# nwihardjo/SpaghettiSearch

Hardware: AMD Instinct MI355X
Metric: pagerank_iters_per_sec (higher is better)
Workload: dtype f64

## Files before the change

spaghettisearch_amd/csrc/pagerank.hip:

```cpp
#include "pr_state.hpp"

#include <algorithm>
#include <chrono>
#include <cmath>
#include <memory>

namespace {


template <int GW>
__device__ __forceinline__ double wave_sum_topic(double v) {
#pragma unroll
    for (int off = GW; off < 64; off <<= 1) v += __shfl_xor(v, off, 64);
    return v;
}

__device__ __forceinline__ double zero_row_rank(const PrParams& p, int sweep, double S, double x0) {
    return ((sweep == 0 ? x0 : 0.0) + p.teleport) / S;
}
__device__ __forceinline__ double teleport_of(const PrParams& p, uint32_t lrow, int t) {
    if (!p.memb || !((p.ts_mask >> t) & 1u)) return p.teleport;
    return ((p.memb[lrow] >> t) & 1u) ? p.tin[t] : 0.0;
}
__device__ __forceinline__ double zero_row_rank_ts(const PrParams& p, int sweep, double S, double x0, double tele) {
// ... 1032 lines not shown
            w.beg = in_ptr[w.row] + w.count * SEGW;
            w.end = min(in_ptr[w.row + 1], w.beg + SEGW);
            break;
        case V_QUAD:
        case V_DEG: w.beg = in_ptr[w.row]; w.end = in_ptr[w.row + w.count]; break;
        default: return;
    }
    work[i] = w;
}

__global__ __launch_bounds__(TPB) void k_pr_remap_src(const uint32_t* __restrict__ in_src, uint32_t* __restrict__ out, size_t n_edges, uint32_t pos_nd,
                                                      uint32_t cnt_nd, const uint32_t* __restrict__ outdeg, const uint32_t* __restrict__ sh_deg,
                                                      uint32_t n_shared, uint32_t zrow) {
    for (size_t e = (size_t)blockIdx.x * TPB + threadIdx.x; e < n_edges; e += (size_t)gridDim.x * TPB) {
        uint32_t w = NT_LOAD(&in_src[e]);
        const uint32_t s = w & SRC_MASK;
        if (s >= pos_nd) {
            uint32_t row = zrow;
            if (s < cnt_nd && n_shared) {
                const uint32_t od = outdeg[s];
                uint32_t lo = 0, hi = n_shared;
                while (lo < hi) {
                    const uint32_t mid = (lo + hi) >> 1;
                    if (sh_deg[mid] < od) lo = mid + 1; else hi = mid;
                }
                if (lo < n_shared && sh_deg[lo] == od) row = zrow + 1 + lo;
            }
            w = (w & ~SRC_MASK) | row;
        }
        NT_STORE(w, &out[e]);
    }
}

template <int GW>
__global__ __launch_bounds__(TPB) void k_pr_begin(PrParams p) {
    const int lane = threadIdx.x & 63;
    const int t = lane % GW;
    const double x0 = p.x0[t];
    double* __restrict__ Tw = p.tab_wr[1];
    double csum = 0.0;
    for (uint32_t i = blockIdx.x * TPB + threadIdx.x; i < p.n_shared * (uint32_t)GW; i += gridDim.x * TPB)
        Tw[(size_t)(p.zrow + 1) * GW + i] = p.d * x0 / (double)p.sh_deg[i / GW];
    const size_t n_el = ((size_t)p.sl_nd + p.sl_d) * GW;
    for (size_t i = (size_t)blockIdx.x * TPB + threadIdx.x; i < n_el; i += (size_t)gridDim.x * TPB) {
        const uint32_t lrow = (uint32_t)(i / GW);
        const bool real = lrow < p.sl_nd ? lrow < p.cnt_nd : (lrow - p.sl_nd) < p.cnt_d;
        p.x[i] = real ? x0 : 0.0;
        if (lrow < p.sl_nd) {
            double c = 0.0;
            if (real) c = p.d * x0 / (double)p.outdeg[lrow];
            if ((p.world == 1 || lrow + 2 < p.sl_nd) && lrow < p.tab_rows) Tw[i] = c;
            csum += c;
        }
    }
    block_reduce_and_publish<GW>(p, 0.0, csum, Tw, true);
}

template <int GW>
__global__ void k_pr_finalize(PrParams p, const double* __restrict__ table, int is_begin) {
    if (threadIdx.x != 0 || blockIdx.x != 0) return;
    if (!is_begin && p.ctl->n_active == 0) return;
    double dl[MAXK], cs[MAXK];
    for (int k = 0; k < MAXK; k++) { dl[k] = 0.0; cs[k] = 0.0; }
    for (int r = 0; r < p.world; r++) {
        const size_t base = ((size_t)r * p.sl_nd + (p.sl_nd - 2)) * GW;
        for (int k = 0; k < GW; k++) {
// ... 235 lines not shown
        } else {
            SS_GW_DISPATCH(GW, sweep_occupancy, &per_cu);
        }
        occ_cache[slot] = per_cu < 1 ? 1 : per_cu;
    }
    return occ_cache[slot];
}
int multi_blocks_per_cu(int gw) {
    static std::mutex occ2_mu;
    static int occ_multi[3] = {0, 0, 0};
    std::lock_guard<std::mutex> lk2(occ2_mu);
    int& occ = occ_multi[gw <= 2 ? gw : 0];
    if (!occ) {
        int o = 0;
        if (gw == 1) (void)hipOccupancyMaxActiveBlocksPerMultiprocessor(&o, k_pr_multi_n<1, 1>, TPB, 0);
        else (void)hipOccupancyMaxActiveBlocksPerMultiprocessor(&o, k_pr_multi_n<2, 1>, TPB, 0);
        occ = std::max(o, 1);
    }
    return occ;
}
unsigned grid_for(const ss_ctx* ctx, ss_pr* pr, const PlanOptions& opt, int per_cu, bool vitems, size_t n_items) {
    per_cu = (int)std::max<int64_t>(1, opt.blocks_per_cu == PlanOptions::AUTO ? per_cu : opt.blocks_per_cu);
    const int64_t want = ctx->opt("pr.persistent", 0);
    pr->persist_mode = want == 2 ? 2 : 1;
    pr->persist = pr->nwave && pr->g->world == 1 && !ctx->opt("pr.affine", 0) && want > 0;
    if (pr->persist) {
        const int admit = std::max(1, multi_blocks_per_cu(pr->gw) - 2);
        per_cu = (int)std::max<int64_t>(1, std::min<int64_t>(std::min(admit, std::max(1, per_cu / 2)), ctx->opt("pr.persistent_blocks", 4)));
    }
    return vitems ? (unsigned)std::min<size_t>(std::max<size_t>(1, ss::div_up(n_items, (size_t)WAVES * opt.items_per_wave)), (size_t)ctx->cu_count * per_cu)
                  : (unsigned)std::min<size_t>(n_items, (size_t)ctx->cu_count * 8);
}

void fill_params(ss_pr* pr, const Cut& cut, const PlanOptions& opt, double damping, double eps, int32_t max_iter, int32_t k_topics) {
    const ss_graph* g = pr->g;
    PrParams& p = pr->prm;
    p.in_ptr = g->in_ptr.p;
    p.in_src = g->in_src.p;
    p.outdeg = g->outdeg.p;
    p.x = pr->x.p;
    if (g->world == 1) {
        p.tab_rd[0] = pr->tab0.p; p.tab_wr[0] = pr->tab1.p;
        p.tab_rd[1] = pr->tab1.p; p.tab_wr[1] = pr->tab0.p;
    } else {
        p.tab_rd[0] = p.tab_rd[1] = pr->tab0.p;
        p.tab_wr[0] = p.tab_wr[1] = pr->send.p;
    }
    p.work = pr->work.p;
    p.partials = pr->partials.p;
    p.segpart = pr->segpart.p;
    p.rowticket = pr->rowticket.p;
    p.ctl = pr->ctl.p;
    p.x0 = pr->x0.p;
    p.d = damping;
    p.teleport = 1.0 - damping;
    p.eps = eps;
    p.tele_n = p.teleport * (double)g->n;
    p.max_iter = max_iter;
    p.k_topics = k_topics;
    p.world = g->world;
    p.sl_nd = g->sl_nd;
    p.cnt_nd = g->cnt_nd;
    p.sl_d = g->sl_d;
    p.cnt_d = g->cnt_d;
    p.seg_edges = cut.seg_edges;
    p.n_items = (uint32_t)cut.items.size();
    p.pos_nd = cut.pos_nd;
    p.pos_d = cut.pos_d;
    p.zrow = (uint32_t)g->nd_int;
    p.tab_rows = g->sl_nd;
    p.woff = pr->woff.p;
    p.stagger_div = opt.stagger != 0 ? (uint32_t)std::max(g->ctx->cu_count, 1) : 0u;
    p.stagger_code = opt.stagger >= 10 ? (uint32_t)(opt.stagger - 10) : 0u;
    p.class_order = pack_class_order(opt.class_order);
    p.n_order = pack_n_order(opt.n_class_order);
}

uint64_t fnv1a(const void* q, size_t n, uint64_t h = 0xcbf29ce484222325ull) {
    const unsigned char* b = static_cast<const unsigned char*>(q);
    for (size_t i = 0; i < n; i++) { h ^= b[i]; h *= 0x100000001b3ull; }
    return h;
}
void trace_plan(const ss_pr* pr, const std::vector<WorkItem>& work, const std::vector<uint32_t>& woff) {
    const PrParams& p = pr->prm;
    const double sd[] = {p.d, p.teleport, p.eps, p.tele_n};
    const uint32_t su[] = {(uint32_t)p.max_iter, (uint32_t)p.k_topics, (uint32_t)p.world, p.sl_nd, p.cnt_nd, p.sl_d, p.cnt_d, p.seg_edges, p.n_items,
                           p.pos_nd, p.pos_d, p.ts_mask, p.zrow, p.stagger_div, p.stagger_code, p.class_order, p.n_order};
    fprintf(stderr, "[pr trace] plan: work %016llx (%zu items)  woff %016llx  params %016llx  nblocks %u\n",
            (unsigned long long)fnv1a(work.data(), work.size() * sizeof(WorkItem)), work.size(),
            (unsigned long long)fnv1a(woff.data(), woff.size() * sizeof(uint32_t)),
            (unsigned long long)fnv1a(su, sizeof(su), fnv1a(sd, sizeof(sd))), pr->nblocks);
}

int32_t alloc_tables(ss_pr* pr, hipStream_t st, size_t rows) {
    const ss_graph* g = pr->g;
    ss_ctx* ctx = g->ctx;
    const size_t GW = (size_t)pr->gw;
    SS_HIP(ctx, pr->tab0.alloc(rows * GW));
    SS_HIP(ctx, hipMemsetAsync(pr->tab0.p, 0, std::max<size_t>(pr->tab0.bytes(), 8), st));
    if (g->world == 1) {
        SS_HIP(ctx, pr->tab1.alloc(rows * GW));
        SS_HIP(ctx, hipMemsetAsync(pr->tab1.p, 0, std::max<size_t>(pr->tab1.bytes(), 8), st));
    } else {
        SS_HIP(ctx, pr->send.alloc((size_t)g->sl_nd * GW));
        SS_HIP(ctx, hipMemsetAsync(pr->send.p, 0, std::max<size_t>(pr->send.bytes(), 8), st));
    }
    return SS_OK;
}
int32_t unshare_rows(ss_pr* pr, hipStream_t st) {
    if (!pr->prm.share) return SS_OK;
    const ss_graph* g = pr->g;
    SS_HIP(g->ctx, hipStreamSynchronize(st));
    SS_TRY(alloc_tables(pr, st, (size_t)g->nd_int + 1));
    pr->src_shared.release();
    pr->sh_deg.release();
    PrParams& p = pr->prm;
    p.tab_rd[0] = pr->tab0.p; p.tab_wr[0] = pr->tab1.p;
    p.tab_rd[1] = pr->tab1.p; p.tab_wr[1] = pr->tab0.p;
    p.in_src = g->in_src.p;
    p.sh_deg = nullptr;
    p.n_shared = 0;
    p.share = 0;
    p.zrow = (uint32_t)g->nd_int;
    p.tab_rows = g->sl_nd;
    return SS_OK;
}

#ifdef SS_PR_WAVETIME
FILE* open_dump(const char* name) {
    const char* dir = getenv("SS_PR_WAVETIME_DIR");
    return fopen((std::string(dir && *dir ? dir : ".") + "/" + name).c_str(), "w");
}
void dump_wave_loads(const Cut& cut, const std::vector<double>& cost, const std::vector<uint32_t>& owner, uint32_t nw) {
    FILE* f = open_dump("pr_load.csv");
    if (!f) return;
    std::vector<double> wl(nw, 0.0), wcls((size_t)nw * 6, 0.0);
    for (size_t i = 0; i < cut.items.size(); i++) {
        int kc = 0; while (kc < 5 && i >= cut.vbeg[kc + 1]) kc++;
        wl[owner[i]] += cost[i]; wcls[(size_t)owner[i] * 6 + kc] += cost[i];
    }
    fprintf(f, "wave,load,c0,c1,c2,c3,c4,c5\n");
    for (uint32_t w = 0; w < nw; w++) fprintf(f, "%u,%.2f,%.2f,%.2f,%.2f,%.2f,%.2f,%.2f\n", w, wl[w], wcls[(size_t)w * 6], wcls[(size_t)w * 6 + 1], wcls[(size_t)w * 6 + 2], wcls[(size_t)w * 6 + 3], wcls[(size_t)w * 6 + 4], wcls[(size_t)w * 6 + 5]);
    fclose(f);
}
void dump_wave_times(const ss_pr* pr) {
    if (pr->gw < 8) return;
    (void)hipDeviceSynchronize();
    const uint32_t nwv = std::min<uint32_t>(65536u, pr->nblocks * WAVES);
    std::vector<unsigned long long> h((size_t)nwv * 2);
    if (hipMemcpyFromSymbol(h.data(), HIP_SYMBOL(g_pr_wt), h.size() * sizeof(unsigned long long)) != hipSuccess || !nwv) return;
    unsigned long long t0 = ~0ull;
    for (uint32_t w = 0; w < nwv; w++) t0 = std::min(t0, h[2 * w]);
    std::vector<double> st(nwv), en(nwv);
    for (uint32_t w = 0; w < nwv; w++) { st[w] = (double)(h[2 * w] - t0) / 100.0; en[w] = (double)(h[2 * w + 1] - t0) / 100.0; }
    std::sort(st.begin(), st.end()); std::sort(en.begin(), en.end());
    if (FILE* f = open_dump("pr_wt.csv")) {
        fprintf(f, "wave,start_us,end_us\n");
        for (uint32_t w = 0; w < nwv; w++) fprintf(f, "%u,%.2f,%.2f\n", w, (double)(h[2 * w] - t0) / 100.0, (double)(h[2 * w + 1] - t0) / 100.0);
        fclose(f);
    }
    fprintf(stderr, "[pr wavetime] %u waves: start us median %.1f max %.1f | out of items us min %.1f p10 %.1f median %.1f p90 %.1f p99 %.1f max %.1f\n", nwv,
            st[nwv / 2], st[nwv - 1], en[0], en[nwv / 10], en[nwv / 2], en[nwv * 9 / 10], en[(size_t)nwv * 99 / 100], en[nwv - 1]);
}
#endif

}

extern "C" {

int32_t ss_pr_create(ss_graph* g, double damping, double eps, int32_t max_iter, int32_t k_topics,
                     const int32_t* n_topic, ss_pr** out) {
    if (!g) return SS_ERR_INVALID;
    ss_ctx* ctx = g->ctx;
    std::lock_guard<std::recursive_mutex> lk(ctx->mu);
    if (!out) return ctx->fail(SS_ERR_INVALID, "ss_pr_create: out is NULL");
    *out = nullptr;
    if (k_topics < 1 || !n_topic) return ctx->fail(SS_ERR_INVALID, "ss_pr_create: k_topics < 1 or n_topic NULL");
    if (k_topics > MAXK) return ctx->fail(SS_ERR_UNSUPPORTED, "ss_pr_create: k_topics %d > %d per state (ss_pagerank_run splits larger K)", k_topics, MAXK);
    SS_HIP(ctx, hipSetDevice(ctx->device));
    hipStream_t st = ctx->stream;

    ss_pr* pr = new (std::nothrow) ss_pr();
    if (!pr) return ctx->fail(SS_ERR_OOM, "ss_pr_create: host OOM");
    std::unique_ptr<ss_pr> guard(pr);
    pr->g = g;
    pr->k = k_topics;
    const bool force_narrow = ctx->opt("pr.force_narrow", 0) != 0;
    pr->gw = pick_gw(k_topics, g->nd_int, force_narrow, ctx->opt("pr.narrow_wave", 1) != 0);
    pr->nwave = pr->gw <= 2 && !force_narrow && ctx->opt("pr.narrow_wave", 1) != 0;
    const int GW = pr->gw;
    const bool vitems = GW >= 8 || pr->nwave;
    const int GI = pr->nwave ? 8 : GW;
    const size_t n_local = g->n_local();
    if (((uint64_t)g->nd_int + 1) * GW * 8 >= (1ull << 32))
        return ctx->fail(SS_ERR_UNSUPPORTED, "ss_pr_create: contribution table of %llu rows x %d topics exceeds 4 GiB (shard the graph over more ranks)",
                         (unsigned long long)g->nd_int, GW);

    const bool trace = ctx->opt("pr.trace", 0) != 0;
    auto t_now = [] { return std::chrono::steady_clock::now(); };
    auto t_ms = [](std::chrono::steady_clock::time_point a, std::chrono::steady_clock::time_point b) { return std::chrono::duration<double, std::milli>(b - a).count(); };
    SS_HIP(ctx, pr->x.alloc(n_local * GW));
    bool share = GW >= 8 && g->world == 1 && ctx->opt("pr.affine", 0) == 0 && ctx->opt("pr.share_zero_rows", 1) != 0;
    if (!share) SS_TRY(alloc_tables(pr, st, (size_t)g->nd_int + 1));

    const auto tc0 = t_now();
    const PlanOptions opt = plan_options(ctx, pr, n_local);
    Cut cut = cut_items(g->h_indeg_nd, g->h_indeg_d, g->sl_nd, GI, pr->nwave, opt);
    const uint32_t n_tail = g->cnt_nd - cut.pos_nd;
    struct PinGuard { ss_ctx* c; void* p = nullptr; size_t cap = 0; ~PinGuard() { c->pin_free(p, cap); } } tail_od{ctx};
    if (share && n_tail == 0) {
        share = false;
        SS_TRY(alloc_tables(pr, st, (size_t)g->nd_int + 1));
    }
    if (share) {
        tail_od.p = ctx->pin_alloc((size_t)n_tail * sizeof(uint32_t), &tail_od.cap);
        if (!tail_od.p) return ctx->fail(SS_ERR_OOM, "ss_pr_create: no pinned host memory for %u out-degrees", n_tail);
        SS_HIP(ctx, hipMemcpyAsync(tail_od.p, g->outdeg.p + cut.pos_nd, (size_t)n_tail * sizeof(uint32_t), hipMemcpyDeviceToHost, st));
    }
    const auto tc1 = t_now();
    const int per_cu = sweep_blocks_per_cu(pr);
    const auto tc1a = t_now();
    pr->nblocks = grid_for(ctx, pr, opt, per_cu, vitems, cut.items.size());
    static const std::vector<uint32_t> no_woff;
    const std::vector<uint32_t>* woff = &no_woff;
    if (vitems) {
        const uint32_t nw = pr->nblocks * WAVES;
        const auto td0 = t_now();
        const std::vector<double>& cost = item_costs(cut, g->h_indeg_nd, g->h_indeg_d, g->sl_nd, GI, pr->nwave);
        const auto td0a = t_now();
        std::vector<uint32_t>& owner = deal_items(cut, cost, nw, pr->nwave, opt);
#ifdef SS_PR_WAVETIME
        dump_wave_loads(cut, cost, owner, nw);
#endif
        const auto td1 = t_now();
        if (trace) fprintf(stderr, "[pr trace]   deal: occupancy query %.2f ms, costs %.3f ms, owners %.3f ms\n", t_ms(tc1, tc1a), t_ms(td0, td0a), t_ms(td0a, td1));
        woff = &place_items(cut, owner, nw);
        if (trace) fprintf(stderr, "[pr trace]   deal: placement %.3f ms\n", t_ms(td1, t_now()));
    }
    const std::vector<WorkItem>& items = cut.items;

    g->settle();
    const auto tc2 = t_now();
    SharedRows sh;
    if (share) {
        SS_HIP(ctx, hipStreamSynchronize(st));
        const auto ts0 = t_now();
        sh = plan_shared_rows(static_cast<const uint32_t*>(tail_od.p), n_tail, cut.pos_nd);
        const auto ts1 = t_now();
        SS_TRY(alloc_tables(pr, st, (size_t)sh.table_rows));
        SS_HIP(ctx, pr->sh_deg.alloc(sh.deg.size()));
        SS_HIP(ctx, hipMemcpyAsync(pr->sh_deg.p, sh.deg.data(), sh.deg.size() * sizeof(uint32_t), hipMemcpyHostToDevice, st));
        SS_HIP(ctx, pr->src_shared.alloc(g->e_local));
        if (g->e_local)
            hipLaunchKernelGGL(k_pr_remap_src, dim3((unsigned)std::min<uint64_t>(ss::div_up(g->e_local, TPB), (uint64_t)ctx->cu_count * 16)), dim3(TPB), 0, st,
                               (const uint32_t*)g->in_src.p, pr->src_shared.p, (size_t)g->e_local, cut.pos_nd, g->cnt_nd, (const uint32_t*)g->outdeg.p,
                               (const uint32_t*)pr->sh_deg.p, (uint32_t)sh.deg.size(), sh.zrow);
        if (trace) fprintf(stderr, "[pr trace]   shared rows: %u rows without in-edges -> %zu shared rows (host %.3f ms), table %llu rows\n", n_tail, sh.deg.size(),
                           t_ms(ts0, ts1), (unsigned long long)sh.table_rows);
    }
    SS_HIP(ctx, pr->partials.alloc(((size_t)std::max(pr->nblocks, ss::begin_blocks(pr)) + 8) * 2 * GW));
    SS_HIP(ctx, pr->segpart.alloc((size_t)std::max(cut.nsegs, 1u) * GW));
    SS_HIP(ctx, pr->rowticket.alloc(std::max(cut.nmulti, 1u)));
    SS_HIP(ctx, hipMemsetAsync(pr->rowticket.p, 0, pr->rowticket.bytes(), st));
    SS_HIP(ctx, pr->woff.alloc(std::max<size_t>(woff->size(), 8)));
    if (!woff->empty()) SS_HIP(ctx, hipMemcpyAsync(pr->woff.p, woff->data(), woff->size() * sizeof(uint32_t), hipMemcpyHostToDevice, st));
    SS_HIP(ctx, pr->work.alloc(items.size()));
    SS_HIP(ctx, hipMemcpyAsync(pr->work.p, items.data(), items.size() * sizeof(WorkItem), hipMemcpyHostToDevice, st));
    if (vitems)
        hipLaunchKernelGGL(k_pr_item_ranges, dim3(ss::div_up(items.size(), TPB)), dim3(TPB), 0, st, pr->work.p, (uint32_t)items.size(), (const uint32_t*)g->in_ptr.p);
    SS_HIP(ctx, pr->ctl.alloc(1));
    SS_HIP(ctx, hipMemsetAsync(pr->ctl.p, 0, sizeof(PrCtl), st));
    double h_x0[MAXK];
    for (int k = 0; k < MAXK; k++) h_x0[k] = k < k_topics ? 1.0 / (double)n_topic[k] : 0.0;
    SS_HIP(ctx, pr->x0.alloc(MAXK));
    SS_HIP(ctx, hipMemcpyAsync(pr->x0.p, h_x0, sizeof(h_x0), hipMemcpyHostToDevice, st));
    SS_HIP(ctx, hipStreamSynchronize(st));
    if (trace) fprintf(stderr, "[pr trace] ss_pr_create: build_work %.2f ms (%zu items), edge ranges + deal %.2f ms, alloc + upload %.2f ms\n", t_ms(tc0, tc1), items.size(), t_ms(tc1, tc2), t_ms(tc2, t_now()));
    if (trace) fprintf(stderr, "[pr trace] where the state lives: x %p  tab0 %p  tab1 %p  in_src %p  in_ptr %p  outdeg %p  work %p  woff %p\n", (void*)pr->x.p, (void*)pr->tab0.p,
                       (void*)pr->tab1.p, (void*)g->in_src.p, (void*)g->in_ptr.p, (void*)g->outdeg.p, (void*)pr->work.p, (void*)pr->woff.p);

    fill_params(pr, cut, opt, damping, eps, max_iter, k_topics);
    if (share) {
        PrParams& p = pr->prm;
        p.in_src = pr->src_shared.p;
        p.sh_deg = pr->sh_deg.p;
        p.n_shared = (uint32_t)sh.deg.size();
        p.share = 1;
        p.zrow = sh.zrow;
        p.tab_rows = cut.pos_nd;
    }
    if (trace) trace_plan(pr, items, *woff);
    g->users++;
    *out = guard.release();
    return SS_OK;
}

int32_t ss_pr_set_teleport(ss_pr* pr, const uint64_t* set_ptr, const uint32_t* set_nodes) {
    if (!pr) return SS_ERR_INVALID;
    ss_ctx* ctx = pr->g->ctx;
    std::lock_guard<std::recursive_mutex> lk(ctx->mu);
    SS_HIP(ctx, hipSetDevice(ctx->device));
    if (pr->begun) return ctx->fail(SS_ERR_STATE, "ss_pr_set_teleport: call before ss_pr_begin");
    hipStream_t st = ctx->stream;
    PrParams& p = pr->prm;
    if (!set_ptr) {
        p.memb = nullptr; p.tin = nullptr; p.nz_in = nullptr; p.ts_mask = 0;
        return SS_OK;
    }
    const ss_graph* g = pr->g;
    const int K = pr->k;
    SS_TRY(unshare_rows(pr, st));
    std::vector<uint64_t> h_ptr(K + 1);
    SS_HIP(ctx, ss::copy_in(ctx->stream, h_ptr.data(), set_ptr, (K + 1) * sizeof(uint64_t)));
    if (h_ptr[0] != 0) return ctx->fail(SS_ERR_INVALID, "ss_pr_set_teleport: set_ptr[0] != 0");
    for (int k = 0; k < K; k++)
        if (h_ptr[k + 1] < h_ptr[k]) return ctx->fail(SS_ERR_INVALID, "ss_pr_set_teleport: set_ptr not non-decreasing");
    const uint64_t total = h_ptr[K];
    if (total && !set_nodes) return ctx->fail(SS_ERR_INVALID, "ss_pr_set_teleport: set_nodes is NULL");
    double h_tin[MAXK];
    uint32_t mask = 0;
    for (int k = 0; k < MAXK; k++) {
        h_tin[k] = 0.0;
        if (k < K && h_ptr[k + 1] > h_ptr[k]) {
            mask |= 1u << k;
            h_tin[k] = p.teleport * (double)g->n / (double)(h_ptr[k + 1] - h_ptr[k]);
        }
    }
// ... 35 lines not shown
    SS_HIP(ctx, hipMemcpyAsync(pr->nz_in.p, h_nz, sizeof(h_nz), hipMemcpyHostToDevice, st));
    SS_HIP(ctx, hipStreamSynchronize(st));
    p.memb = pr->memb.p;
    p.tin = pr->tin.p;
    p.nz_in = pr->nz_in.p;
    p.ts_mask = mask;
    return SS_OK;
}

int32_t ss_pr_destroy(ss_pr* pr) {
#ifdef SS_PR_WAVETIME
    if (pr) dump_wave_times(pr);
#endif

    if (!pr) return SS_ERR_INVALID;
    ss_ctx* ctx = pr->g->ctx;
    std::lock_guard<std::recursive_mutex> lk(ctx->mu);
    (void)hipSetDevice(ctx->device);
    if (!ss::device_wedged(ctx->device)) {
        (void)hipStreamSynchronize(ctx->stream);
        (void)hipStreamSynchronize(ctx->comm_stream);
    }
    pr->g->users--;
    delete pr;
    return SS_OK;
}

int32_t ss_pr_begin(ss_pr* pr) {
    if (!pr) return SS_ERR_INVALID;
    ss_ctx* ctx = pr->g->ctx;
    std::lock_guard<std::recursive_mutex> lk(ctx->mu);
    SS_HIP(ctx, hipSetDevice(ctx->device));
    if (pr->need_finalize) return ctx->fail(SS_ERR_STATE, "ss_pr_begin: pending exchange/finalize");
    SS_HIP(ctx, hipMemsetAsync(&pr->ctl.p->ticket, 0, sizeof(uint32_t), ctx->stream));
    ss::pr_launch_begin(pr, ctx->stream, ss::begin_blocks(pr));
    SS_HIP(ctx, hipGetLastError());
    pr->begun = true;
    if (pr->g->world > 1) {
        pr->need_finalize = true;
        pr->finalize_is_begin = true;
    }
    return SS_OK;
}

int32_t ss_pr_step(ss_pr* pr, int32_t n_steps) {
    if (!pr) return SS_ERR_INVALID;
    ss_ctx* ctx = pr->g->ctx;
    std::lock_guard<std::recursive_mutex> lk(ctx->mu);
    SS_HIP(ctx, hipSetDevice(ctx->device));
    if (!pr->begun) return ctx->fail(SS_ERR_STATE, "ss_pr_step: ss_pr_begin not called");
    if (pr->need_finalize) return ctx->fail(SS_ERR_STATE, "ss_pr_step: pending exchange/finalize");
    if (n_steps < 1) return ctx->fail(SS_ERR_INVALID, "ss_pr_step: n_steps < 1");
    if (pr->g->world > 1 && n_steps != 1) return ctx->fail(SS_ERR_INVALID, "ss_pr_step: world>1 needs an exchange after every step");
    SS_HIP(ctx, hipEventRecord(ctx->ev[0][0], ctx->stream));
    if (pr->persist && !pr->prm.memb && !pr->prm.aff) {
        SS_GW_DISPATCH(pr->gw, launch_multi, pr, ctx->stream, (int)n_steps);
    } else {
        for (int i = 0; i < n_steps; i++) ss::pr_launch_step(pr, ctx->stream);
    }
    SS_HIP(ctx, hipEventRecord(ctx->ev[0][1], ctx->stream));
    ctx->ev_valid[0] = true;
    SS_HIP(ctx, hipGetLastError());
    if (pr->g->world > 1) {
        pr->need_finalize = true;
        pr->finalize_is_begin = false;
    }
    return SS_OK;
}

int32_t ss_pr_finalize(ss_pr* pr) {
// ... 156 lines not shown
```

spaghettisearch_amd/csrc/pagerank_run.hip:

```cpp
#include "pr_state.hpp"

#include <algorithm>

namespace {

constexpr int AFF_KC = 16;
__global__ __launch_bounds__(TPB) void k_aff_delta(const double2* __restrict__ xp, const double2* __restrict__ xn, const AffCtl* __restrict__ a,
                                                   uint32_t sl_nd, uint32_t pos_nd, uint32_t pos_d, double* __restrict__ partials) {
    __shared__ double red[WAVES][AFF_KC];
    if (a->n_active == 0) return;
    const int k_real = a->k_real;
    const double r_old = a->r_prev, r_new = a->r_x, s_old = a->s_prev, s_new = a->s_x;
    const uint32_t n_rows = pos_nd + pos_d;
    const int lane = threadIdx.x & 63, wave = threadIdx.x >> 6;
    for (int k0 = 0; k0 < k_real; k0 += AFF_KC) {
        double u[AFF_KC], d_old[AFF_KC], d_new[AFF_KC], acc[AFF_KC];
        bool any = false;
#pragma unroll
        for (int j = 0; j < AFF_KC; j++) {
            const bool on = k0 + j < k_real && a->active[k0 + j] != 0;
            any = any || on;
            u[j] = on ? a->u[k0 + j] : 0.0;
            d_old[j] = on ? r_old * u[j] + s_old : 1.0;
            d_new[j] = on ? r_new * u[j] + s_new : 1.0;
// ... 629 lines not shown
        for (int k = 0; k < k_topics && rc == SS_OK; k++)
            for (size_t i = 0; i < n_rows; i++) rank_out[(size_t)k * n + ids[i]] = part[(size_t)k * n_rows + i];
    }
    for (int s = 0; s < world && rc == SS_OK && !affine; s++) {
        const size_t n_rows = (size_t)shards[s]->cnt_nd + shards[s]->cnt_d;
        std::vector<uint32_t> ids(n_rows);
        for (int b = 0; b < B && rc == SS_OK; b++) {
            const int kb = k0[b + 1] - k0[b];
            std::vector<double> part((size_t)kb * n_rows);
            rc = ss_pr_read_local(sh[s].blk[b], ids.data(), part.data());
            if (rc != SS_OK) break;
            for (int k = 0; k < kb; k++)
                for (size_t i = 0; i < n_rows; i++) rank_out[(size_t)(k0[b] + k) * n + ids[i]] = part[(size_t)k * n_rows + i];
        }
    }
    for (auto& s : sh)
        for (ss_pr* pr : s.blk) ss_pr_destroy(pr);
    return rc;
}

int32_t ss_pagerank_run(ss_graph* g, double damping, double eps, int32_t max_iter, int32_t k_topics,
                        const int32_t* n_topic, double* rank_out, int32_t* iters_out) {
    if (!g) return SS_ERR_INVALID;
    ss_ctx* ctx = g->ctx;
    std::lock_guard<std::recursive_mutex> lk(ctx->mu);
    if (g->world != 1) return ctx->fail(SS_ERR_STATE, "ss_pagerank_run: needs a (rank 0, world 1) graph");
    if (k_topics < 1 || k_topics > SS_MAX_TOPICS || !n_topic || !rank_out)
        return ctx->fail(SS_ERR_INVALID, "ss_pagerank_run: bad k_topics / NULL argument");
    SS_TRY(check_eps(ctx, "ss_pagerank_run", eps, max_iter));
    if (ctx->opt("pr.affine", 0) != 0) return run_affine(g, damping, eps, max_iter, k_topics, n_topic, rank_out, iters_out);
    for (int k0 = 0; k0 < k_topics; k0 += MAXK) {
        const int kk = std::min(MAXK, k_topics - k0);
        ss_pr* pr = nullptr;
        SS_TRY(ss_pr_create(g, damping, eps, max_iter, kk, n_topic + k0, &pr));
        int32_t rc = ss_pr_begin(pr);
        int32_t n_active = kk, sweeps = 0;
        const int BATCH = 8;
        while (rc == SS_OK && n_active > 0) {
            int todo = BATCH;
            if (max_iter > 0) todo = std::min(BATCH, std::max(1, max_iter - sweeps));
            rc = ss_pr_step(pr, todo);
            if (rc == SS_OK) rc = ss_pr_status(pr, iters_out ? iters_out + k0 : nullptr, &n_active, &sweeps, nullptr, nullptr);
        }
        if (rc == SS_OK) rc = ss_pr_read(pr, rank_out + (size_t)k0 * g->n);
        ss_pr_destroy(pr);
        if (rc != SS_OK) return rc;
    }
    return SS_OK;
}

}
```

spaghettisearch_amd/csrc/pr_plan.hpp:

```cpp
#pragma once
#include "sorted_degrees.hpp"

#include <algorithm>
#include <cstdint>
#include <utility>
#include <vector>

namespace {

constexpr int TPB = 256;
constexpr int WAVES = TPB / 64;
constexpr int CH = 16;
constexpr uint32_t SEGW = 2048;

enum : uint32_t { W_SEG = 0, W_WAVE = 1, W_GROUP = 2, W_ZERO = 3,
                  V_SEG = 8,
                  V_ROWW = 9,
                  V_QUAD = 10,
                  V_DEG = 11,
                  V_ZERO = 12 };

struct WorkItem {
    uint32_t kind;
    uint32_t row;
// ... 219 lines not shown
            c0 = c1;
        }
    }
    for (size_t i0 = 0; i0 < n_items; i0 += nw) {
        const size_t n_chunk = std::min<size_t>(nw, n_items - i0);
        if (i0 && snake) {
            std::reverse(by_load.begin(), by_load.end());
        } else if (i0) {
            key.resize(nw);
            for (uint32_t w = 0; w < nw; w++) key[w] = {load[w], w};
            std::sort(key.begin(), key.end());
            for (uint32_t w = 0; w < nw; w++) by_load[w] = key[w].second;
        }
        idx.resize(n_chunk);
        for (size_t j = 0; j < n_chunk; j++) idx[j] = global_order ? order[i0 + j] : (uint32_t)(i0 + j);
        const auto falling = [&](uint32_t a, uint32_t b) { return cost[a] > cost[b]; };
        size_t run_end = 0, n_merge = 0;
        for (size_t j = 1; j <= n_chunk && !global_order; j++) {
            if (j < n_chunk && !(cost[i0 + j] > cost[i0 + j - 1])) continue;
            if (run_end) {
                if (++n_merge > 8) { std::stable_sort(idx.begin(), idx.end(), falling); break; }
                std::inplace_merge(idx.begin(), idx.begin() + (ptrdiff_t)run_end, idx.begin() + (ptrdiff_t)j, falling);
            }
            run_end = j;
        }
        for (size_t j = 0; j < n_chunk; j++) {
            owner[idx[j]] = by_load[j];
            load[by_load[j]] += cost[idx[j]];
        }
    }
    return owner;
}

inline const std::vector<uint32_t>& place_items(Cut& cut, std::vector<uint32_t>& owner, uint32_t nw) {
    PlanScratch& s = plan_scratch();
    auto& items = cut.items;
    auto &woff = s.woff, &cnt = s.cnt;
    woff.assign((size_t)nw * 8, 0);
    cnt.assign((size_t)nw * 8, 0);
    for (int k = 0; k < 6; k++) {
        const size_t i1 = k < 5 ? std::min<size_t>(cut.vbeg[k + 1], items.size()) : items.size();
        for (size_t i = std::min<size_t>(cut.vbeg[k], i1); i < i1; i++) { owner[i] = owner[i] * 8 + (uint32_t)k; cnt[owner[i]]++; }
    }
    uint32_t run_off = 0;
    for (uint32_t w = 0; w < nw; w++) {
        for (int k = 0; k < 8; k++) {
            woff[(size_t)w * 8 + k] = run_off;
            run_off += cnt[(size_t)w * 8 + k];
            cnt[(size_t)w * 8 + k] = woff[(size_t)w * 8 + k];
        }
    }
    s.dealt.resize(items.size());
    for (size_t i = 0; i < items.size(); i++) s.dealt[cnt[owner[i]]++] = items[i];
    s.dealt.push_back({V_ZERO, 0, 0, 0, 0, 0, 0, 0});
    s.dealt.push_back({V_ZERO, 0, 0, 0, 0, 0, 0, 0});
    items.swap(s.dealt);
    return woff;
}

inline uint32_t pack_class_order(int64_t code) {
    uint32_t packed = 0, seen = 0;
    for (int pos = 5; pos >= 0; pos--) {
        const uint32_t c = (uint32_t)(code % 10);
        code /= 10;
        packed |= (c & 7u) << (3 * pos);
        if (c < 6) seen |= 1u << c;
    }
    return seen == 0x3Fu ? packed : (0u | 1u << 3 | 2u << 6 | 3u << 9 | 4u << 12 | 5u << 15);
}
inline uint32_t pack_n_order(int64_t code) {
    uint32_t packed = 0, seen = 0;
    for (int pos = 3; pos >= 0; pos--) {
        const uint32_t c = (uint32_t)(code % 10);
        code /= 10;
        packed |= (c & 3u) << (2 * pos);
        if (c < 4) seen |= 1u << c;
    }
    return seen == 0xFu ? packed : (0u | 1u << 2 | 2u << 4 | 3u << 6);
}

struct SharedRows {
    std::vector<uint32_t> deg;
    uint32_t zrow = 0;
    uint32_t base = 0;
    uint64_t table_rows = 0;
    uint32_t row_of(uint32_t od) const {
        const auto it = std::lower_bound(deg.begin(), deg.end(), od);
        return it != deg.end() && *it == od ? base + (uint32_t)(it - deg.begin()) : zrow;
    }
};
inline SharedRows plan_shared_rows(const uint32_t* od, size_t n, uint32_t pos_nd) {
    SharedRows sh;
    uint32_t hi = 0;
    for (size_t i = 0; i < n; i++) hi = std::max(hi, od[i]);
    if (n && (uint64_t)hi <= 4 * (uint64_t)n + 65536) {
        std::vector<unsigned char> seen((size_t)hi + 1, 0);
        for (size_t i = 0; i < n; i++) seen[od[i]] = 1;
        for (size_t v = 0; v <= hi; v++)
            if (seen[v]) sh.deg.push_back((uint32_t)v);
    } else if (n) {
        sh.deg.assign(od, od + n);
        std::sort(sh.deg.begin(), sh.deg.end());
        sh.deg.erase(std::unique(sh.deg.begin(), sh.deg.end()), sh.deg.end());
    }
    sh.zrow = pos_nd;
    sh.base = pos_nd + 1;
    sh.table_rows = (uint64_t)pos_nd + 1 + sh.deg.size();
    return sh;
}

}
```

spaghettisearch_amd/csrc/pr_state.hpp:

```cpp
#pragma once
#include "graph.hpp"
#include "pr_plan.hpp"

namespace {

constexpr int MAXK = 16;

struct PrCtl {
    double S[MAXK];
    double delta[MAXK];
    double csum[MAXK];
    double xz[MAXK];
    double xz_in[MAXK];
    double tele[MAXK];
    int32_t active[MAXK];
    int32_t iters[MAXK];
    int32_t sweep;
    int32_t n_active;
    uint32_t ticket;
    uint32_t stuck;
    uint32_t gticket[8];
};

constexpr int AFF_MAXK = 256;
// ... 34 lines not shown
    uint32_t stagger_div;
    uint32_t stagger_code;
    uint32_t class_order;
    uint32_t n_order;
    double* x_alt;
    AffCtl* aff;
    const double* tele_col;
    const uint32_t* sh_deg;
    uint32_t n_shared;
    uint32_t share;
    uint32_t tab_rows;
};

}

struct ss_pr {
    ss_graph* g = nullptr;
    int gw = 1;
    ss::DevBuf<float> wire_send, wire_recv;
    bool nwave = false;
    int persist_mode = 1;
    bool persist = false;
    int k = 1;
    PrParams prm{};
    unsigned nblocks = 0;
    ss::DevBuf<double> x, tab0, tab1, send, partials, segpart, x0;
    ss::DevBuf<uint32_t> rowticket;
    ss::DevBuf<uint32_t> memb;
    ss::DevBuf<double> tin, nz_in;
    ss::DevBuf<WorkItem> work;
    ss::DevBuf<uint32_t> woff;
    ss::DevBuf<uint32_t> src_shared;
    ss::DevBuf<uint32_t> sh_deg;
    ss::DevBuf<PrCtl> ctl;
    bool begun = false;
    bool need_finalize = false;
    bool finalize_is_begin = false;
};

#pragma GCC visibility push(hidden)
namespace ss {
unsigned begin_blocks(const ss_pr* pr);
void pr_launch_begin(ss_pr* pr, hipStream_t st, unsigned nb);
void pr_launch_step(ss_pr* pr, hipStream_t st);
void pr_launch_finalize(ss_pr* pr, hipStream_t st, int is_begin);
size_t pr_wire_floats(const ss_pr* pr);
hipError_t pr_wire_alloc(ss_pr* pr);
void pr_wire_pack(ss_pr* pr, hipStream_t st);
void pr_wire_unpack(ss_pr* pr, hipStream_t st);
}
#pragma GCC visibility pop

namespace {
inline int32_t read_ctl(ss_ctx* ctx, const ss_pr* pr, hipStream_t st, const char* what, const PrCtl** out) {
    ctx->pin_used = 0;
    PrCtl* const hp = ctx->pin<PrCtl>();
    if (hipMemcpyAsync(hp, pr->ctl.p, sizeof(PrCtl), hipMemcpyDeviceToHost, st) != hipSuccess) return ctx->fail(SS_ERR_HIP, "%s: status read failed", what);
    SS_TRY(ss::sync_bounded(ctx, st, what));
    *out = hp;
    return SS_OK;
}
}
```

Baseline: 18440.

## Overlap PageRank setup with GPU work and compute tail degrees on device

The create path now builds the set of distinct tail out-degrees with a shared-memory bitmap kernel, so the host reads back a small bitmap instead of every tail out-degree. It falls back to the full copy when a degree is too large for the bitmap. It also enqueues the begin kernel before the host deals work items, writes the plan straight into pinned memory, uploads it asynchronously, and memsets only the unshared part of the rank tables. The goal is to cut host-side setup and synchronisation latency. The cost is more complex lifetime handling for the pinned plan buffer, which the destructor now frees.

New measurement: 18430. Within noise of the previous version (-0.0%).

```diff
diff --git a/spaghettisearch_amd/csrc/pagerank.hip b/spaghettisearch_amd/csrc/pagerank.hip
--- a/spaghettisearch_amd/csrc/pagerank.hip
+++ b/spaghettisearch_amd/csrc/pagerank.hip
@@ -1088,6 +1088,21 @@
     }
 }
 
+constexpr uint32_t SH_SEEN_BITS = 1u << 16, SH_SEEN_WORDS = SH_SEEN_BITS / 32;
+__global__ __launch_bounds__(TPB) void k_pr_tail_degrees(const uint32_t* __restrict__ od, uint32_t n, uint32_t* __restrict__ seen) {
+    __shared__ uint32_t s_seen[SH_SEEN_WORDS + 1];
+    for (uint32_t i = threadIdx.x; i <= SH_SEEN_WORDS; i += TPB) s_seen[i] = 0u;
+    __syncthreads();
+    for (uint32_t i = blockIdx.x * TPB + threadIdx.x; i < n; i += gridDim.x * TPB) {
+        const uint32_t d = od[i];
+        if (d < SH_SEEN_BITS) atomicOr(&s_seen[d >> 5], 1u << (d & 31u));
+        else s_seen[SH_SEEN_WORDS] = 1u;
+    }
+    __syncthreads();
+    for (uint32_t i = threadIdx.x; i <= SH_SEEN_WORDS; i += TPB)
+        if (s_seen[i]) atomicOr(&seen[i], s_seen[i]);
+}
+
 template <int GW>
 __global__ __launch_bounds__(TPB) void k_pr_begin(PrParams p) {
     const int lane = threadIdx.x & 63;
@@ -1389,7 +1404,7 @@
                   : (unsigned)std::min<size_t>(n_items, (size_t)ctx->cu_count * 8);
 }
 
-void fill_params(ss_pr* pr, const Cut& cut, const PlanOptions& opt, double damping, double eps, int32_t max_iter, int32_t k_topics) {
+void fill_params(ss_pr* pr, const Cut& cut, uint32_t n_items, const PlanOptions& opt, double damping, double eps, int32_t max_iter, int32_t k_topics) {
     const ss_graph* g = pr->g;
     PrParams& p = pr->prm;
     p.in_ptr = g->in_ptr.p;
@@ -1421,7 +1436,7 @@
     p.sl_d = g->sl_d;
     p.cnt_d = g->cnt_d;
     p.seg_edges = cut.seg_edges;
-    p.n_items = (uint32_t)cut.items.size();
+    p.n_items = n_items;
     p.pos_nd = cut.pos_nd;
     p.pos_d = cut.pos_d;
     p.zrow = (uint32_t)g->nd_int;
@@ -1438,26 +1453,27 @@
     for (size_t i = 0; i < n; i++) { h ^= b[i]; h *= 0x100000001b3ull; }
     return h;
 }
-void trace_plan(const ss_pr* pr, const std::vector<WorkItem>& work, const std::vector<uint32_t>& woff) {
+void trace_plan(const ss_pr* pr, const WorkItem* work, size_t n_work, const uint32_t* woff, size_t n_woff) {
     const PrParams& p = pr->prm;
     const double sd[] = {p.d, p.teleport, p.eps, p.tele_n};
     const uint32_t su[] = {(uint32_t)p.max_iter, (uint32_t)p.k_topics, (uint32_t)p.world, p.sl_nd, p.cnt_nd, p.sl_d, p.cnt_d, p.seg_edges, p.n_items,
                            p.pos_nd, p.pos_d, p.ts_mask, p.zrow, p.stagger_div, p.stagger_code, p.class_order, p.n_order};
     fprintf(stderr, "[pr trace] plan: work %016llx (%zu items)  woff %016llx  params %016llx  nblocks %u\n",
-            (unsigned long long)fnv1a(work.data(), work.size() * sizeof(WorkItem)), work.size(),
-            (unsigned long long)fnv1a(woff.data(), woff.size() * sizeof(uint32_t)),
+            (unsigned long long)fnv1a(work, n_work * sizeof(WorkItem)), n_work,
+            (unsigned long long)fnv1a(woff, n_woff * sizeof(uint32_t)),
             (unsigned long long)fnv1a(su, sizeof(su), fnv1a(sd, sizeof(sd))), pr->nblocks);
 }
 
-int32_t alloc_tables(ss_pr* pr, hipStream_t st, size_t rows) {
+int32_t alloc_tables(ss_pr* pr, hipStream_t st, size_t rows, size_t zero_from = 0) {
     const ss_graph* g = pr->g;
     ss_ctx* ctx = g->ctx;
     const size_t GW = (size_t)pr->gw;
+    const size_t off = std::min(zero_from, rows) * GW, zbytes = std::max<size_t>((rows * GW - off) * sizeof(double), 8);
     SS_HIP(ctx, pr->tab0.alloc(rows * GW));
-    SS_HIP(ctx, hipMemsetAsync(pr->tab0.p, 0, std::max<size_t>(pr->tab0.bytes(), 8), st));
+    SS_HIP(ctx, hipMemsetAsync(pr->tab0.p + off, 0, zbytes, st));
     if (g->world == 1) {
         SS_HIP(ctx, pr->tab1.alloc(rows * GW));
-        SS_HIP(ctx, hipMemsetAsync(pr->tab1.p, 0, std::max<size_t>(pr->tab1.bytes(), 8), st));
+        SS_HIP(ctx, hipMemsetAsync(pr->tab1.p + off, 0, zbytes, st));
     } else {
         SS_HIP(ctx, pr->send.alloc((size_t)g->sl_nd * GW));
         SS_HIP(ctx, hipMemsetAsync(pr->send.p, 0, std::max<size_t>(pr->send.bytes(), 8), st));
@@ -1523,10 +1539,14 @@
 
 }
 
-extern "C" {
-
-int32_t ss_pr_create(ss_graph* g, double damping, double eps, int32_t max_iter, int32_t k_topics,
-                     const int32_t* n_topic, ss_pr** out) {
+namespace ss {
+void pr_enqueue_begin(ss_pr* pr, hipStream_t st) {
+    (void)hipMemsetAsync(&pr->ctl.p->ticket, 0, sizeof(uint32_t), st);
+    pr_launch_begin(pr, st, begin_blocks(pr));
+    pr->begun = true;
+}
+
+int32_t pr_create(ss_graph* g, double damping, double eps, int32_t max_iter, int32_t k_topics, const int32_t* n_topic, bool begin_now, ss_pr** out) {
     if (!g) return SS_ERR_INVALID;
     ss_ctx* ctx = g->ctx;
     std::lock_guard<std::recursive_mutex> lk(ctx->mu);
@@ -1569,74 +1589,74 @@
         share = false;
         SS_TRY(alloc_tables(pr, st, (size_t)g->nd_int + 1));
     }
+    constexpr size_t seen_bytes = (SH_SEEN_WORDS + 1) * sizeof(uint32_t);
     if (share) {
-        tail_od.p = ctx->pin_alloc((size_t)n_tail * sizeof(uint32_t), &tail_od.cap);
-        if (!tail_od.p) return ctx->fail(SS_ERR_OOM, "ss_pr_create: no pinned host memory for %u out-degrees", n_tail);
-        SS_HIP(ctx, hipMemcpyAsync(tail_od.p, g->outdeg.p + cut.pos_nd, (size_t)n_tail * sizeof(uint32_t), hipMemcpyDeviceToHost, st));
-    }
+        tail_od.p = ctx->pin_alloc(seen_bytes, &tail_od.cap);
+        if (!tail_od.p) return ctx->fail(SS_ERR_OOM, "ss_pr_create: no pinned host memory for the out-degree bitmap");
+        SS_HIP(ctx, pr->sh_seen.alloc(SH_SEEN_WORDS + 1));
+        SS_HIP(ctx, hipMemsetAsync(pr->sh_seen.p, 0, seen_bytes, st));
+        hipLaunchKernelGGL(k_pr_tail_degrees, dim3(std::min<unsigned>(ss::div_up(n_tail, TPB * 8), (unsigned)ctx->cu_count * 4)), dim3(TPB), 0, st,
+                           (const uint32_t*)g->outdeg.p + cut.pos_nd, n_tail, pr->sh_seen.p);
+        SS_HIP(ctx, hipMemcpyAsync(tail_od.p, pr->sh_seen.p, seen_bytes, hipMemcpyDeviceToHost, st));
+    }
+    SS_HIP(ctx, pr->segpart.alloc((size_t)std::max(cut.nsegs, 1u) * GW));
+    SS_HIP(ctx, pr->rowticket.alloc(std::max(cut.nmulti, 1u)));
+    SS_HIP(ctx, hipMemsetAsync(pr->rowticket.p, 0, pr->rowticket.bytes(), st));
+    SS_HIP(ctx, pr->ctl.alloc(1));
+    SS_HIP(ctx, hipMemsetAsync(pr->ctl.p, 0, sizeof(PrCtl), st));
+    SS_HIP(ctx, pr->x0.alloc(MAXK));
     const auto tc1 = t_now();
     const int per_cu = sweep_blocks_per_cu(pr);
     const auto tc1a = t_now();
     pr->nblocks = grid_for(ctx, pr, opt, per_cu, vitems, cut.items.size());
-    static const std::vector<uint32_t> no_woff;
-    const std::vector<uint32_t>* woff = &no_woff;
-    if (vitems) {
-        const uint32_t nw = pr->nblocks * WAVES;
-        const auto td0 = t_now();
-        const std::vector<double>& cost = item_costs(cut, g->h_indeg_nd, g->h_indeg_d, g->sl_nd, GI, pr->nwave);
-        const auto td0a = t_now();
-        std::vector<uint32_t>& owner = deal_items(cut, cost, nw, pr->nwave, opt);
-#ifdef SS_PR_WAVETIME
-        dump_wave_loads(cut, cost, owner, nw);
-#endif
-        const auto td1 = t_now();
-        if (trace) fprintf(stderr, "[pr trace]   deal: occupancy query %.2f ms, costs %.3f ms, owners %.3f ms\n", t_ms(tc1, tc1a), t_ms(td0, td0a), t_ms(td0a, td1));
-        woff = &place_items(cut, owner, nw);
-        if (trace) fprintf(stderr, "[pr trace]   deal: placement %.3f ms\n", t_ms(td1, t_now()));
-    }
-    const std::vector<WorkItem>& items = cut.items;
-
-    g->settle();
-    const auto tc2 = t_now();
+    SS_HIP(ctx, pr->partials.alloc(((size_t)std::max(pr->nblocks, ss::begin_blocks(pr)) + 8) * 2 * GW));
+    const uint32_t nw = vitems ? pr->nblocks * WAVES : 0;
+    const std::vector<double>* cost = nullptr;
+    if (vitems) cost = &item_costs(cut, g->h_indeg_nd, g->h_indeg_d, g->sl_nd, GI, pr->nwave);
+    const auto tc1b = t_now();
+
     SharedRows sh;
     if (share) {
+        g->settle();
         SS_HIP(ctx, hipStreamSynchronize(st));
-        const auto ts0 = t_now();
-        sh = plan_shared_rows(static_cast<const uint32_t*>(tail_od.p), n_tail, cut.pos_nd);
-        const auto ts1 = t_now();
-        SS_TRY(alloc_tables(pr, st, (size_t)sh.table_rows));
+        if (static_cast<const uint32_t*>(tail_od.p)[SH_SEEN_WORDS] == 0) {
+            sh = shared_rows_from_bitmap(static_cast<const uint32_t*>(tail_od.p), SH_SEEN_WORDS, cut.pos_nd);
+        } else {
+            ctx->pin_free(tail_od.p, tail_od.cap);
+            tail_od.p = ctx->pin_alloc((size_t)n_tail * sizeof(uint32_t), &tail_od.cap);
+            if (!tail_od.p) return ctx->fail(SS_ERR_OOM, "ss_pr_create: no pinned host memory for %u out-degrees", n_tail);
+            SS_HIP(ctx, hipMemcpyAsync(tail_od.p, g->outdeg.p + cut.pos_nd, (size_t)n_tail * sizeof(uint32_t), hipMemcpyDeviceToHost, st));
+            SS_HIP(ctx, hipStreamSynchronize(st));
+            sh = plan_shared_rows(static_cast<const uint32_t*>(tail_od.p), n_tail, cut.pos_nd);
+        }
+    }
+    const auto tc1c = t_now();
+    const size_t n_up = cut.items.size() + (vitems ? 2 : 0), n_woff = (size_t)nw * 8;
+    const size_t plan_bytes = n_up * sizeof(WorkItem) + n_woff * sizeof(uint32_t) + MAXK * sizeof(double) + sh.deg.size() * sizeof(uint32_t);
+    pr->h_plan = ctx->pin_alloc(plan_bytes, &pr->h_plan_cap);
+    if (!pr->h_plan) return ctx->fail(SS_ERR_OOM, "ss_pr_create: no pinned host memory for the plan (%zu bytes)", plan_bytes);
+    WorkItem* const h_work = static_cast<WorkItem*>(pr->h_plan);
+    uint32_t* const h_woff = reinterpret_cast<uint32_t*>(h_work + n_up);
+    double* const h_x0 = reinterpret_cast<double*>(h_woff + n_woff);
+    uint32_t* const h_shdeg = reinterpret_cast<uint32_t*>(h_x0 + MAXK);
+    for (int k = 0; k < MAXK; k++) h_x0[k] = k < k_topics ? 1.0 / (double)n_topic[k] : 0.0;
+    SS_HIP(ctx, hipMemcpyAsync(pr->x0.p, h_x0, MAXK * sizeof(double), hipMemcpyHostToDevice, st));
+    if (share) {
+        SS_TRY(alloc_tables(pr, st, (size_t)sh.table_rows, (size_t)sh.zrow));
+        std::copy(sh.deg.begin(), sh.deg.end(), h_shdeg);
         SS_HIP(ctx, pr->sh_deg.alloc(sh.deg.size()));
-        SS_HIP(ctx, hipMemcpyAsync(pr->sh_deg.p, sh.deg.data(), sh.deg.size() * sizeof(uint32_t), hipMemcpyHostToDevice, st));
+        SS_HIP(ctx, hipMemcpyAsync(pr->sh_deg.p, h_shdeg, sh.deg.size() * sizeof(uint32_t), hipMemcpyHostToDevice, st));
         SS_HIP(ctx, pr->src_shared.alloc(g->e_local));
         if (g->e_local)
             hipLaunchKernelGGL(k_pr_remap_src, dim3((unsigned)std::min<uint64_t>(ss::div_up(g->e_local, TPB), (uint64_t)ctx->cu_count * 16)), dim3(TPB), 0, st,
                                (const uint32_t*)g->in_src.p, pr->src_shared.p, (size_t)g->e_local, cut.pos_nd, g->cnt_nd, (const uint32_t*)g->outdeg.p,
                                (const uint32_t*)pr->sh_deg.p, (uint32_t)sh.deg.size(), sh.zrow);
-        if (trace) fprintf(stderr, "[pr trace]   shared rows: %u rows without in-edges -> %zu shared rows (host %.3f ms), table %llu rows\n", n_tail, sh.deg.size(),
-                           t_ms(ts0, ts1), (unsigned long long)sh.table_rows);
-    }
-    SS_HIP(ctx, pr->partials.alloc(((size_t)std::max(pr->nblocks, ss::begin_blocks(pr)) + 8) * 2 * GW));
-    SS_HIP(ctx, pr->segpart.alloc((size_t)std::max(cut.nsegs, 1u) * GW));
-    SS_HIP(ctx, pr->rowticket.alloc(std::max(cut.nmulti, 1u)));
-    SS_HIP(ctx, hipMemsetAsync(pr->rowticket.p, 0, pr->rowticket.bytes(), st));
-    SS_HIP(ctx, pr->woff.alloc(std::max<size_t>(woff->size(), 8)));
-    if (!woff->empty()) SS_HIP(ctx, hipMemcpyAsync(pr->woff.p, woff->data(), woff->size() * sizeof(uint32_t), hipMemcpyHostToDevice, st));
-    SS_HIP(ctx, pr->work.alloc(items.size()));
-    SS_HIP(ctx, hipMemcpyAsync(pr->work.p, items.data(), items.size() * sizeof(WorkItem), hipMemcpyHostToDevice, st));
-    if (vitems)
-        hipLaunchKernelGGL(k_pr_item_ranges, dim3(ss::div_up(items.size(), TPB)), dim3(TPB), 0, st, pr->work.p, (uint32_t)items.size(), (const uint32_t*)g->in_ptr.p);
-    SS_HIP(ctx, pr->ctl.alloc(1));
-    SS_HIP(ctx, hipMemsetAsync(pr->ctl.p, 0, sizeof(PrCtl), st));
-    double h_x0[MAXK];
-    for (int k = 0; k < MAXK; k++) h_x0[k] = k < k_topics ? 1.0 / (double)n_topic[k] : 0.0;
-    SS_HIP(ctx, pr->x0.alloc(MAXK));
-    SS_HIP(ctx, hipMemcpyAsync(pr->x0.p, h_x0, sizeof(h_x0), hipMemcpyHostToDevice, st));
-    SS_HIP(ctx, hipStreamSynchronize(st));
-    if (trace) fprintf(stderr, "[pr trace] ss_pr_create: build_work %.2f ms (%zu items), edge ranges + deal %.2f ms, alloc + upload %.2f ms\n", t_ms(tc0, tc1), items.size(), t_ms(tc1, tc2), t_ms(tc2, t_now()));
-    if (trace) fprintf(stderr, "[pr trace] where the state lives: x %p  tab0 %p  tab1 %p  in_src %p  in_ptr %p  outdeg %p  work %p  woff %p\n", (void*)pr->x.p, (void*)pr->tab0.p,
-                       (void*)pr->tab1.p, (void*)g->in_src.p, (void*)g->in_ptr.p, (void*)g->outdeg.p, (void*)pr->work.p, (void*)pr->woff.p);
-
-    fill_params(pr, cut, opt, damping, eps, max_iter, k_topics);
+        if (trace) fprintf(stderr, "[pr trace]   shared rows: %u rows without in-edges -> %zu shared rows (wait + host %.3f ms), table %llu rows\n", n_tail, sh.deg.size(),
+                           t_ms(tc1b, tc1c), (unsigned long long)sh.table_rows);
+    }
+    SS_HIP(ctx, pr->woff.alloc(std::max<size_t>(n_woff, 8)));
+    SS_HIP(ctx, pr->work.alloc(n_up));
+    fill_params(pr, cut, (uint32_t)n_up, opt, damping, eps, max_iter, k_topics);
     if (share) {
         PrParams& p = pr->prm;
         p.in_src = pr->src_shared.p;
@@ -1646,10 +1666,45 @@
         p.zrow = sh.zrow;
         p.tab_rows = cut.pos_nd;
     }
-    if (trace) trace_plan(pr, items, *woff);
+    if (begin_now) pr_enqueue_begin(pr, st);
+    SS_HIP(ctx, hipGetLastError());
+    const auto tc2 = t_now();
+    if (vitems) {
+        std::vector<uint32_t>& owner = deal_items(cut, *cost, nw, pr->nwave, opt);
+#ifdef SS_PR_WAVETIME
+        dump_wave_loads(cut, *cost, owner, nw);
+#endif
+        const auto td1 = t_now();
+        if (trace) fprintf(stderr, "[pr trace]   deal: occupancy query %.2f ms, costs %.3f ms, owners %.3f ms\n", t_ms(tc1, tc1a), t_ms(tc1a, tc1b), t_ms(tc2, td1));
+        place_items_into(cut, owner, nw, h_work, h_woff);
+        if (trace) fprintf(stderr, "[pr trace]   deal: placement %.3f ms\n", t_ms(td1, t_now()));
+    } else {
+        std::copy(cut.items.begin(), cut.items.end(), h_work);
+    }
+    if (!share) g->settle();
+    const auto tc3 = t_now();
+    if (n_woff) SS_HIP(ctx, hipMemcpyAsync(pr->woff.p, h_woff, n_woff * sizeof(uint32_t), hipMemcpyHostToDevice, st));
+    SS_HIP(ctx, hipMemcpyAsync(pr->work.p, h_work, n_up * sizeof(WorkItem), hipMemcpyHostToDevice, st));
+    if (vitems)
+        hipLaunchKernelGGL(k_pr_item_ranges, dim3(ss::div_up(n_up, TPB)), dim3(TPB), 0, st, pr->work.p, (uint32_t)n_up, (const uint32_t*)g->in_ptr.p);
+    SS_HIP(ctx, hipGetLastError());
+    if (trace) fprintf(stderr, "[pr trace] ss_pr_create: build_work %.2f ms (%zu items), grid + costs %.2f ms, shared rows + their enqueues %.2f ms, deal %.2f ms, alloc + upload enqueued %.2f ms\n",
+                       t_ms(tc0, tc1), n_up, t_ms(tc1, tc1b), t_ms(tc1b, tc2), t_ms(tc2, tc3), t_ms(tc3, t_now()));
+    if (trace) fprintf(stderr, "[pr trace] where the state lives: x %p  tab0 %p  tab1 %p  in_src %p  in_ptr %p  outdeg %p  work %p  woff %p\n", (void*)pr->x.p, (void*)pr->tab0.p,
+                       (void*)pr->tab1.p, (void*)g->in_src.p, (void*)g->in_ptr.p, (void*)g->outdeg.p, (void*)pr->work.p, (void*)pr->woff.p);
+
+    if (trace) trace_plan(pr, h_work, n_up, h_woff, n_woff);
     g->users++;
     *out = guard.release();
     return SS_OK;
+}
+}
+
+extern "C" {
+
+int32_t ss_pr_create(ss_graph* g, double damping, double eps, int32_t max_iter, int32_t k_topics,
+                     const int32_t* n_topic, ss_pr** out) {
+    return ss::pr_create(g, damping, eps, max_iter, k_topics, n_topic, false, out);
 }
 
 int32_t ss_pr_set_teleport(ss_pr* pr, const uint64_t* set_ptr, const uint32_t* set_nodes) {
@@ -1751,10 +1806,8 @@
     std::lock_guard<std::recursive_mutex> lk(ctx->mu);
     SS_HIP(ctx, hipSetDevice(ctx->device));
     if (pr->need_finalize) return ctx->fail(SS_ERR_STATE, "ss_pr_begin: pending exchange/finalize");
-    SS_HIP(ctx, hipMemsetAsync(&pr->ctl.p->ticket, 0, sizeof(uint32_t), ctx->stream));
-    ss::pr_launch_begin(pr, ctx->stream, ss::begin_blocks(pr));
+    ss::pr_enqueue_begin(pr, ctx->stream);
     SS_HIP(ctx, hipGetLastError());
-    pr->begun = true;
     if (pr->g->world > 1) {
         pr->need_finalize = true;
         pr->finalize_is_begin = true;
diff --git a/spaghettisearch_amd/csrc/pagerank_run.hip b/spaghettisearch_amd/csrc/pagerank_run.hip
--- a/spaghettisearch_amd/csrc/pagerank_run.hip
+++ b/spaghettisearch_amd/csrc/pagerank_run.hip
@@ -685,8 +685,8 @@
     for (int k0 = 0; k0 < k_topics; k0 += MAXK) {
         const int kk = std::min(MAXK, k_topics - k0);
         ss_pr* pr = nullptr;
-        SS_TRY(ss_pr_create(g, damping, eps, max_iter, kk, n_topic + k0, &pr));
-        int32_t rc = ss_pr_begin(pr);
+        SS_TRY(ss::pr_create(g, damping, eps, max_iter, kk, n_topic + k0, true, &pr));
+        int32_t rc = SS_OK;
         int32_t n_active = kk, sweeps = 0;
         const int BATCH = 8;
         while (rc == SS_OK && n_active > 0) {
diff --git a/spaghettisearch_amd/csrc/pr_plan.hpp b/spaghettisearch_amd/csrc/pr_plan.hpp
--- a/spaghettisearch_amd/csrc/pr_plan.hpp
+++ b/spaghettisearch_amd/csrc/pr_plan.hpp
@@ -275,30 +275,32 @@
     return owner;
 }
 
-inline const std::vector<uint32_t>& place_items(Cut& cut, std::vector<uint32_t>& owner, uint32_t nw) {
+inline void place_items_into(const Cut& cut, std::vector<uint32_t>& owner, uint32_t nw, WorkItem* dealt, uint32_t* woff) {
     PlanScratch& s = plan_scratch();
-    auto& items = cut.items;
-    auto &woff = s.woff, &cnt = s.cnt;
-    woff.assign((size_t)nw * 8, 0);
+    const auto& items = cut.items;
+    auto& cnt = s.cnt;
     cnt.assign((size_t)nw * 8, 0);
     for (int k = 0; k < 6; k++) {
         const size_t i1 = k < 5 ? std::min<size_t>(cut.vbeg[k + 1], items.size()) : items.size();
         for (size_t i = std::min<size_t>(cut.vbeg[k], i1); i < i1; i++) { owner[i] = owner[i] * 8 + (uint32_t)k; cnt[owner[i]]++; }
     }
     uint32_t run_off = 0;
-    for (uint32_t w = 0; w < nw; w++) {
-        for (int k = 0; k < 8; k++) {
-            woff[(size_t)w * 8 + k] = run_off;
-            run_off += cnt[(size_t)w * 8 + k];
-            cnt[(size_t)w * 8 + k] = woff[(size_t)w * 8 + k];
-        }
-    }
-    s.dealt.resize(items.size());
-    for (size_t i = 0; i < items.size(); i++) s.dealt[cnt[owner[i]]++] = items[i];
-    s.dealt.push_back({V_ZERO, 0, 0, 0, 0, 0, 0, 0});
-    s.dealt.push_back({V_ZERO, 0, 0, 0, 0, 0, 0, 0});
-    items.swap(s.dealt);
-    return woff;
+    for (size_t q = 0; q < (size_t)nw * 8; q++) {
+        woff[q] = run_off;
+        run_off += cnt[q];
+        cnt[q] = woff[q];
+    }
+    for (size_t i = 0; i < items.size(); i++) dealt[cnt[owner[i]]++] = items[i];
+    dealt[items.size()] = {V_ZERO, 0, 0, 0, 0, 0, 0, 0};
+    dealt[items.size() + 1] = {V_ZERO, 0, 0, 0, 0, 0, 0, 0};
+}
+inline const std::vector<uint32_t>& place_items(Cut& cut, std::vector<uint32_t>& owner, uint32_t nw) {
+    PlanScratch& s = plan_scratch();
+    s.dealt.resize(cut.items.size() + 2);
+    s.woff.resize((size_t)nw * 8);
+    place_items_into(cut, owner, nw, s.dealt.data(), s.woff.data());
+    cut.items.swap(s.dealt);
+    return s.woff;
 }
 
 inline uint32_t pack_class_order(int64_t code) {
@@ -351,5 +353,14 @@
     sh.table_rows = (uint64_t)pos_nd + 1 + sh.deg.size();
     return sh;
 }
-
-}
+inline SharedRows shared_rows_from_bitmap(const uint32_t* seen, size_t words, uint32_t pos_nd) {
+    SharedRows sh;
+    for (size_t w = 0; w < words; w++)
+        for (uint32_t bits = seen[w]; bits; bits &= bits - 1) sh.deg.push_back((uint32_t)(w * 32) + (uint32_t)__builtin_ctz(bits));
+    sh.zrow = pos_nd;
+    sh.base = pos_nd + 1;
+    sh.table_rows = (uint64_t)pos_nd + 1 + sh.deg.size();
+    return sh;
+}
+
+}
diff --git a/spaghettisearch_amd/csrc/pr_state.hpp b/spaghettisearch_amd/csrc/pr_state.hpp
--- a/spaghettisearch_amd/csrc/pr_state.hpp
+++ b/spaghettisearch_amd/csrc/pr_state.hpp
@@ -90,7 +90,17 @@
     ss::DevBuf<uint32_t> woff;
     ss::DevBuf<uint32_t> src_shared;
     ss::DevBuf<uint32_t> sh_deg;
+    ss::DevBuf<uint32_t> sh_seen;
     ss::DevBuf<PrCtl> ctl;
+    void* h_plan = nullptr;
+    size_t h_plan_cap = 0;
+    ~ss_pr() {
+        if (!h_plan) return;
+        ss_ctx* ctx = g->ctx;
+        if (ss::device_wedged(ctx->device)) return;
+        (void)hipStreamSynchronize(ctx->stream);
+        ctx->pin_free(h_plan, h_plan_cap);
+    }
     bool begun = false;
     bool need_finalize = false;
     bool finalize_is_begin = false;
@@ -102,6 +112,8 @@
 void pr_launch_begin(ss_pr* pr, hipStream_t st, unsigned nb);
 void pr_launch_step(ss_pr* pr, hipStream_t st);
 void pr_launch_finalize(ss_pr* pr, hipStream_t st, int is_begin);
+void pr_enqueue_begin(ss_pr* pr, hipStream_t st);
+int32_t pr_create(ss_graph* g, double damping, double eps, int32_t max_iter, int32_t k_topics, const int32_t* n_topic, bool begin_now, ss_pr** out);
 size_t pr_wire_floats(const ss_pr* pr);
 hipError_t pr_wire_alloc(ss_pr* pr);
 void pr_wire_pack(ss_pr* pr, hipStream_t st);
```
